# ecpoppenheimer/TensorFlowRayTrace

Measured on AMD Instinct MI355X. Metric: ray-surface intersection tests/sec (fwd+bwd), higher is better.
Workload: dtype f32 ray state, f32 filter + f64 decisions

## Files before the change

### tensorflowraytrace_amd/csrc/tfrt_trace3d.hip

```cpp
#include <vector>

#include <type_traits>
#include "tfrt_common.h"
#include "goal_finish.h"
#include "wave_schedule.h"

namespace tfrt {

constexpr int TILE = 512;
constexpr int KC = 24;

constexpr int ERR_CAPACITY = 1;


__global__ __launch_bounds__(BLOCK) void k_center(const double* __restrict__ fverts, int M,
                                                  double* __restrict__ c0, int32_t* nrays0, int n,
                                                  int32_t* tail8, unsigned int* scan_ticket) {
  if (nrays0 != nullptr) {
    if (threadIdx.x == 0) *nrays0 = n;
    if (threadIdx.x < 8) tail8[threadIdx.x] = 0;
    if (threadIdx.x == 0 && scan_ticket != nullptr) *scan_ticket = 0u;
  }
  __shared__ double red[WAVES][3];
  __shared__ double ctr[3];
// ... 2473 lines not shown
  if (p == a.P && a.P > 0 && a.unfinished != nullptr) {
    const unsigned long long m = __ballot(alive);
    if (alive) {
      const int slot = a.wbase[(size_t)(a.P - 1) * a.wstride + qwave].x + rank_below(m);
      const T* rin = a.rays_ws + (size_t)(a.P - 1) * 6 * a.n;
#pragma unroll
      for (int k = 0; k < 6; ++k) a.unfinished[(int64_t)k * a.N + slot] = rin[k * a.n + i];
      if (a.unfinished_id != nullptr) a.unfinished_id[slot] = rid;
    }
  }
}


template <typename G>
__device__ __forceinline__ void add6(const G* g, int64_t cap, int64_t slot, double a[3],
                                     double b[3]) {
  if (g == nullptr) return;
  for (int k = 0; k < 3; ++k) {
    a[k] += static_cast<double>(g[k * cap + slot]);
    b[k] += static_cast<double>(g[(3 + k) * cap + slot]);
  }
}

template <typename T>
struct SweepStore {
  using type = float;
};
template <>
struct SweepStore<double> {
  using type = double;
};

template <typename T>
__device__ __forceinline__ int backward_ray(
    int i, const T* __restrict__ rays_in, int64_t stride_in, const int32_t* __restrict__ ray_id_in,
    const int32_t* __restrict__ rec_tri, const double* __restrict__ rec_t,
    const uint8_t* __restrict__ rec_cls, const int32_t* __restrict__ rec_slot,
    const int32_t* __restrict__ pass_counts, const tfrt_scene3d& sc, double L, double dead_len,
    const typename SweepStore<T>::type* __restrict__ g_child, int64_t child_stride,
    const double* __restrict__ g_fin, int64_t cap_fin, const double* __restrict__ g_act,
    int64_t cap_act, const double* __restrict__ g_stp, int64_t cap_stp,
    const double* __restrict__ g_dead, int64_t cap_dead,
    typename SweepStore<T>::type* __restrict__ g_out, double* __restrict__ g_src_out,
    int64_t out_stride, double gP[9]);

template <int CTRL>
__device__ __forceinline__ double dpp_f64(const double v) {
  const long long b = __double_as_longlong(v);
  const int lo = __builtin_amdgcn_update_dpp(0, (int)(b & 0xFFFFFFFFll), CTRL, 0xF, 0xF, false);
  const int hi = __builtin_amdgcn_update_dpp(0, (int)(b >> 32), CTRL, 0xF, 0xF, false);
  return __longlong_as_double(((long long)hi << 32) | (unsigned int)lo);
}

constexpr int WSUM_SLOTS = 32, WSUM_CELLS = 576;
__device__ __forceinline__ void wave_face_sums(int tri, const double gP[9], double* wacc,
                                               int32_t* wface, double* __restrict__ g_fverts) {
  const int lane = threadIdx.x & 63;
  int slot = -1, ns = 0;
  unsigned long long todo = __ballot(tri >= 0);
  if (todo == 0ull) return;
  while (todo != 0ull && ns < WSUM_SLOTS) {
    const int leader = __ffsll((long long)todo) - 1;
    const int k = __builtin_amdgcn_readlane(tri, leader);
    const bool mine = tri == k;
    if (mine) slot = ns;
    if (lane == leader) wface[ns] = k;
    ++ns;
    todo &= ~__ballot(mine);
  }
  const int copies = ns <= 8 ? 8 : (ns <= 16 ? 4 : 2);
  const int cells = ns * 9 * copies;
  for (int k = lane; k < cells; k += 64) wacc[k] = 0.0;
  wave_fence();
  if (tri >= 0) {
    if (slot >= 0) {
      double* w = &wacc[slot * 9 * copies + (lane & (copies - 1))];
#pragma unroll
      for (int c = 0; c < 9; ++c)
        if (gP[c] != 0.0) unsafeAtomicAdd(w + c * copies, gP[c]);
    } else {
      double* gp = g_fverts + 9 * (int64_t)tri;
#pragma unroll
      for (int c = 0; c < 9; ++c)
        if (gP[c] != 0.0) unsafeAtomicAdd(gp + c, gP[c]);
    }
  }
  wave_fence();
  for (int k0 = 0; k0 < cells; k0 += 64) {
    const int k = k0 + lane;
    double v = k < cells ? wacc[k] : 0.0;
    v += dpp_f64<0xB1>(v);
    if (copies >= 4) v += dpp_f64<0x4E>(v);
    if (copies >= 8) v += dpp_f64<0x141>(v);
    if ((lane & (copies - 1)) == 0 && k < cells && v != 0.0) {
      const int term = k / copies;
      unsafeAtomicAdd(g_fverts + 9 * (int64_t)wface[term / 9] + (term % 9), v);
    }
  }
  wave_fence();
}

template <typename T, int BW>
__global__ __launch_bounds__(64 * BW) void k_backward3d(
    const T* __restrict__ rays_in, int64_t stride_in, const int32_t* __restrict__ n_ptr,
    const int32_t* __restrict__ ray_id_in, const int32_t* __restrict__ rec_tri,
    const double* __restrict__ rec_t, const uint8_t* __restrict__ rec_cls,
    const int32_t* __restrict__ rec_slot, const int32_t* __restrict__ pass_counts,
    tfrt_scene3d sc, double L, double dead_len,
    const typename SweepStore<T>::type* __restrict__ g_child, int64_t child_stride,
    const double* __restrict__ g_fin, int64_t cap_fin, const double* __restrict__ g_act,
    int64_t cap_act, const double* __restrict__ g_stp, int64_t cap_stp,
    const double* __restrict__ g_dead, int64_t cap_dead,
    typename SweepStore<T>::type* __restrict__ g_out, double* __restrict__ g_src_out,
    int64_t out_stride, double* __restrict__ g_fverts,
    typename SweepStore<T>::type* __restrict__ stash_g, int32_t* __restrict__ stash_face,
    int wave_sums) {
  const int n = *n_ptr;
  const int q0 = blockIdx.x * (64 * BW) + threadIdx.x;
  const int i = q0;
  if (wave_sums) {
    if ((q0 & ~63) >= n) return;
    __shared__ double wacc[BW][WSUM_CELLS];
    __shared__ int32_t wface[BW][WSUM_SLOTS];
    const int wave = threadIdx.x >> 6;
    double gP[9];
    int tri = -1;
    if (i < n)
      tri = backward_ray<T>(i, rays_in, stride_in, ray_id_in, rec_tri, rec_t, rec_cls, rec_slot,
                            pass_counts, sc, L, dead_len, g_child, child_stride, g_fin, cap_fin,
                            g_act, cap_act, g_stp, cap_stp, g_dead, cap_dead, g_out, g_src_out,
                            out_stride, gP);
    wave_face_sums(tri, gP, wacc[wave], wface[wave], g_fverts);
    return;
  }
  if (i >= n) return;
  double gP[9];
  const int tri = backward_ray<T>(i, rays_in, stride_in, ray_id_in, rec_tri, rec_t, rec_cls,
                                  rec_slot, pass_counts, sc, L, dead_len, g_child, child_stride,
                                  g_fin, cap_fin, g_act, cap_act, g_stp, cap_stp, g_dead, cap_dead,
                                  g_out, g_src_out, out_stride, gP);
  if (stash_face != nullptr) {
    stash_face[i] = tri;
    if (tri >= 0) {
      using S = typename SweepStore<T>::type;
      S* o = stash_g + 9 * (int64_t)i;
#pragma unroll
      for (int c = 0; c < 9; ++c) o[c] = static_cast<S>(gP[c]);
    }
    return;
  }
  if (tri >= 0) {
    double* gp = g_fverts + 9 * (int64_t)tri;
#pragma unroll
    for (int c = 0; c < 9; ++c) {
      if (gP[c] != 0.0) unsafeAtomicAdd(gp + c, gP[c]);
    }
  }
}

constexpr int FACE_WINDOW = 2048;

template <typename S>
__global__ __launch_bounds__(1024) void k_face_accumulate(
    const int32_t* __restrict__ nrays, int passes, int64_t pass_stride,
    const int32_t* __restrict__ stash_face, const S* __restrict__ stash_g, int chunk, int M,
    double* __restrict__ g_fverts) {
  __shared__ double acc[FACE_WINDOW * 9];
  const int lo = blockIdx.x * chunk;
  if (lo >= nrays[0]) return;
  const int w0 = blockIdx.y * FACE_WINDOW;
  const int w1 = min(M, w0 + FACE_WINDOW);
  for (int k = threadIdx.x; k < FACE_WINDOW * 9; k += 1024) acc[k] = 0.0;
  __syncthreads();
  for (int p = 0; p < passes; ++p) {
    const int hi = min(nrays[p], lo + chunk);
    const int32_t* __restrict__ face = stash_face + (int64_t)p * pass_stride;
    const S* __restrict__ terms = stash_g + 9 * (int64_t)p * pass_stride;
// ... 152 lines not shown
      const double dl = (dead_len != 0.0) ? dead_len : 1.0;
      for (int k = 0; k < 3; ++k) {
        gs[k] = a[k] + (1.0 - dl) * b[k];
        ge[k] = dl * b[k];
      }
    }
  } else {
    double g_s[3] = {0, 0, 0}, g_h[3] = {0, 0, 0}, g_ce[3] = {0, 0, 0};
    bool has_child = false;
    if (cls == CLS_FINISHED) {
      if (seed_fin != nullptr) {
        for (int k = 0; k < 3; ++k) {
          g_s[k] += seed_fin[k];
          g_h[k] += seed_fin[3 + k];
        }
      } else {
        add6(g_fin, cap_fin, slot, g_s, g_h);
      }
    } else if (cls == CLS_STOPPED) {
      add6(g_stp, cap_stp, slot, g_s, g_h);
    } else {
      if (g_act != nullptr)
        add6(g_act, cap_act, (slot_global ? 0 : (int64_t)pass_counts[4 + CLS_ACTIVE]) + slot, g_s, g_h);
      if (child_pass) {
        has_child = true;
        for (int k = 0; k < 3; ++k) {
          g_h[k] += child[k];
          g_ce[k] += child[3 + k];
        }
      }
    }
    bool nz = has_child;
    for (int k = 0; k < 3; ++k) nz = nz || g_s[k] != 0.0 || g_h[k] != 0.0;
    if (nz) {
      if (!early) {
        if (tri_known < -1) tri = rec_tri[i];
        load_face(has_child);
      }
      double gn[2];
      const bool want_n = GN && has_child && sc.grad_n_in != nullptr && sc.n_table == nullptr;
      const int branch = ((tape & TAPE_INTERNAL) ? 1 : 0) | ((tape & TAPE_REFLECT) ? 2 : 0);
      adjoint3d(s, e, P, t_rec, has_child, n_in, n_out, L, g_s, g_h, g_ce, gs, ge, gP, gn, branch,
                want_n);
      if (want_n) {
        if (gn[0] != 0.0) unsafeAtomicAdd(sc.grad_n_in + tri, gn[0]);
        if (gn[1] != 0.0) unsafeAtomicAdd(sc.grad_n_out + tri, gn[1]);
      }
      if (sc.face_grad_mask == nullptr || sc.face_grad_mask[tri] != 0) face_out = tri;
    }
  }
  return face_out;
}

__device__ __forceinline__ int backward_core_loaded(
    int tape, int tri, bool child_pass, const double s[3], const double e[3], const double P[9],
    double t_rec, double n_in, double n_out, bool face_wanted, double L, const double child[6],
    const double seed[6], double gs[3], double ge[3], double gP[9]) {
  int face_out = -1;
  const int cls = tape & 3;
  for (int k = 0; k < 3; ++k) gs[k] = ge[k] = 0.0;
  if (cls != CLS_DEAD) {
    double g_s[3] = {0, 0, 0}, g_h[3] = {0, 0, 0}, g_ce[3] = {0, 0, 0};
    bool has_child = false;
    if (cls == CLS_FINISHED) {
      for (int k = 0; k < 3; ++k) {
        g_s[k] += seed[k];
        g_h[k] += seed[3 + k];
      }
    } else if (cls == CLS_ACTIVE && child_pass) {
      has_child = true;
      for (int k = 0; k < 3; ++k) {
        g_h[k] += child[k];
        g_ce[k] += child[3 + k];
      }
    }
    bool nz = has_child;
    for (int k = 0; k < 3; ++k) nz = nz || g_s[k] != 0.0 || g_h[k] != 0.0;
    if (nz) {
      const int branch = ((tape & TAPE_INTERNAL) ? 1 : 0) | ((tape & TAPE_REFLECT) ? 2 : 0);
      adjoint3d(s, e, P, t_rec, has_child, n_in, n_out, L, g_s, g_h, g_ce, gs, ge, gP, nullptr,
                branch, false);
      if (face_wanted) face_out = tri;
    }
  }
  return face_out;
}

template <typename T>
__device__ __forceinline__ int backward_ray(
    int i, const T* __restrict__ rays_in, int64_t stride_in, const int32_t* __restrict__ ray_id_in,
    const int32_t* __restrict__ rec_tri, const double* __restrict__ rec_t,
    const uint8_t* __restrict__ rec_cls, const int32_t* __restrict__ rec_slot,
    const int32_t* __restrict__ pass_counts, const tfrt_scene3d& sc, double L, double dead_len,
    const typename SweepStore<T>::type* __restrict__ g_child, int64_t child_stride,
    const double* __restrict__ g_fin, int64_t cap_fin, const double* __restrict__ g_act,
    int64_t cap_act, const double* __restrict__ g_stp, int64_t cap_stp,
    const double* __restrict__ g_dead, int64_t cap_dead,
    typename SweepStore<T>::type* __restrict__ g_out, double* __restrict__ g_src_out,
    int64_t out_stride, double gP[9]) {
  const int tape = rec_cls[i];
  const int slot = rec_slot[i];
  double child[6] = {0, 0, 0, 0, 0, 0};
  const bool child_pass = g_child != nullptr;
  if (child_pass && (tape & 3) == CLS_ACTIVE) {
    for (int k = 0; k < 6; ++k) child[k] = static_cast<double>(g_child[k * child_stride + slot]);
  }
  double gs[3], ge[3];
  const int face_out = backward_core<T>(i, tape, slot, rays_in, stride_in, ray_id_in, rec_tri,
                                        rec_t, pass_counts, sc, L, dead_len, child_pass, child,
                                        nullptr, g_fin, cap_fin, g_act, cap_act, g_stp, cap_stp, g_dead,
                                        cap_dead, gs, ge, gP);
  if (g_out != nullptr) {
    using G = typename SweepStore<T>::type;
    for (int k = 0; k < 3; ++k) {
      g_out[k * out_stride + i] = static_cast<G>(gs[k]);
      g_out[(3 + k) * out_stride + i] = static_cast<G>(ge[k]);
    }
  } else if (g_src_out != nullptr) {
    for (int k = 0; k < 3; ++k) {
      g_src_out[k * out_stride + i] = gs[k];
      g_src_out[(3 + k) * out_stride + i] = ge[k];
    }
  }
  return face_out;
}

constexpr int CHAIN_MAXP = 8;

template <typename T>
struct ChainArgs {
  const T* src;
  int64_t src_stride;
  const T* rays_ws;
  const int32_t* nrays;
  const int32_t* rayid;
  const int32_t* rec_tri;
  const int32_t* rec_slot;
  const double* rec_t;
  const uint8_t* rec_cls;
  const int32_t* counts;
  int64_t n;
  int32_t P;
  double L, dead_len;
  const double *g_fin, *g_act, *g_stp, *g_dead;
  int64_t cap_fin, cap_act, cap_stp, cap_dead;
  double* g_src;
  int64_t N;
  double* g_fverts;
  const T* fin_rays;
  int64_t fin_cap;
  GoalFields gf;
  const double* goal;
  int64_t goal_stride, goal_ray_stride;
  double* partial;
  int32_t* partial_cnt;
  const double* feta;
  int32_t inplace;
  int32_t chain_in_lds;
};

#ifndef TFRT_CHAIN_WAVES
#define TFRT_CHAIN_WAVES 4
#endif
template <typename T, int BW, bool GOAL, bool GN>
__global__ __launch_bounds__(64 * BW)
__attribute__((amdgpu_waves_per_eu(TFRT_CHAIN_WAVES, TFRT_CHAIN_WAVES))) void k_backward_chain(
    ChainArgs<T> a, tfrt_scene3d sc) {
#pragma clang fp contract(off)
  const int n0 = a.nrays[0];
  const int i0 = blockIdx.x * (64 * BW) + threadIdx.x;
  if ((i0 & ~63) >= n0) {
    if (GOAL && (threadIdx.x & 63) == 0) {
      a.partial[i0 >> 6] = 0.0;
      if (a.partial_cnt != nullptr) a.partial_cnt[2 * (i0 >> 6)] = a.partial_cnt[2 * (i0 >> 6) + 1] = 0;
    }
    return;
  }
  __shared__ double wacc[BW][WSUM_CELLS];
  __shared__ int32_t wface[BW][WSUM_SLOTS];
  extern __shared__ int4 chain_lds[];
  const int lane = threadIdx.x & 63, wave = threadIdx.x >> 6;
  const int P = a.P;
  int4* chain = chain_lds + (size_t)wave * P * 64;
  int last = -1;
  if (i0 < n0) {
    int j = i0;
    for (int p = 0; p < P; ++p) {
      const size_t at = (size_t)p * a.n + j;
      const int tape = a.rec_cls[at], tri = a.rec_tri[at];
      const int slot = a.inplace >= 2 ? j : a.rec_slot[at];
      if (a.chain_in_lds) chain[p * 64 + lane] = make_int4(j, tape, slot, tri);
      last = p;
      if ((tape & 3) != CLS_ACTIVE || p == P - 1) break;
      if (!a.inplace) j = slot;
    }
  }
  int top = last;
#pragma unroll
  for (int d = 32; d > 0; d >>= 1) top = max(top, __shfl_xor(top, d, 64));
  double child[6] = {0, 0, 0, 0, 0, 0};
  double err = 0.0;
  int n_fin = 0, n_entered = 0;
  for (int p = top; p >= 0; --p) {
    double gP[9];
    int tri = -1;
    bool fin_here = false;
    if (p <= last) {
      int4 rec;
      if (a.chain_in_lds) {
        rec = chain[p * 64 + lane];
      } else {
        const size_t at = (size_t)p * a.n + i0;
        rec = make_int4(i0, a.rec_cls[at], a.inplace >= 2 ? i0 : a.rec_slot[at], a.rec_tri[at]);
      }
      const int j = rec.x, tape = rec.y, slot = rec.z;
      const size_t off = (size_t)p * a.n;
      const T* rin = p == 0 ? a.src : a.rays_ws + (size_t)(p - 1) * 6 * a.n;
      const int64_t sin = p == 0 ? a.src_stride : a.n;
      const int32_t* idin = (p == 0 || a.inplace) ? nullptr : a.rayid + (size_t)(p - 1) * a.n;
      double seed[6] = {0, 0, 0, 0, 0, 0};
      if (GOAL && p == last && (tape & 3) == CLS_FINISHED) {
        fin_here = true;
        double fin_row[6] = {0, 0, 0, 0, 0, 0};
        if (a.inplace) {
          double s0[3], e0[3], h0[3];
          load_ray3(rin, sin, j, s0, e0);
          hit_point(s0, e0, a.rec_t[off + j], h0);
#pragma unroll
          for (int k = 0; k < 3; ++k) {
            fin_row[k] = s0[k];
            fin_row[3 + k] = static_cast<double>(static_cast<T>(h0[k]));
          }
        }
        for (int c = 0; c < a.gf.n; ++c) {
          const int row = a.gf.row[c];
          double out_c = 0.0;
// ... 21 lines not shown
                             rec.w, a.feta, a.inplace != 0);
      for (int k = 0; k < 3; ++k) {
        child[k] = gs[k];
        child[3 + k] = ge[k];
      }
    }
    if (GOAL) {
      n_fin += __popcll(__ballot(fin_here));
      n_entered += __popcll(__ballot(p <= last));
    }
    wave_face_sums(tri, gP, wacc[wave], wface[wave], a.g_fverts);
  }
  if (a.g_src != nullptr && i0 < n0) {
    for (int k = 0; k < 6; ++k) a.g_src[k * a.N + i0] = child[k];
  }
  if (GOAL) {
#pragma unroll
    for (int d = 32; d > 0; d >>= 1) err += __shfl_xor(err, d, 64);
    if (lane == 0) {
      a.partial[i0 >> 6] = err;
      if (a.partial_cnt != nullptr) {
        a.partial_cnt[2 * (i0 >> 6)] = n_fin;
        a.partial_cnt[2 * (i0 >> 6) + 1] = n_entered;
      }
    }
  }
}

template <typename T>
struct ChainGoalArgs {
  const T* src;
  int64_t src_stride;
  const T* rays_ws;
  const int32_t* nrays;
  const int32_t* rec_tri;
  const double* rec_t;
  const uint8_t* rec_cls;
  int64_t n;
  int32_t P;
  double L;
  double* g_src;
  int64_t N;
  double* g_fverts;
  GoalFields gf;
  const double* goal;
  int64_t goal_stride, goal_ray_stride;
  double* partial;
  int32_t* partial_cnt;
  const double* feta;
  const double* face_verts;
  const uint8_t* face_grad_mask;
  const int32_t* sched;
  int32_t ngroups;
};

template <typename T>
__global__ __launch_bounds__(64)
__attribute__((amdgpu_waves_per_eu(TFRT_CHAIN_WAVES, TFRT_CHAIN_WAVES))) void k_backward_chain_goal_inplace(
    ChainGoalArgs<T> a) {
#pragma clang fp contract(off)
  const int n0 = a.nrays[0];
  int wave = blockIdx.x;
  if (a.sched != nullptr) {
    wave = __builtin_amdgcn_readfirstlane(a.sched[blockIdx.x]);
    if ((unsigned)wave >= (unsigned)a.ngroups) return;
  }
  const int i0 = wave * 64 + threadIdx.x;
  const int lane = threadIdx.x;
  if ((i0 & ~63) >= n0) {
    if (lane == 0) {
      a.partial[i0 >> 6] = 0.0;
      if (a.partial_cnt != nullptr) a.partial_cnt[2 * (i0 >> 6)] = a.partial_cnt[2 * (i0 >> 6) + 1] = 0;
    }
    return;
  }
  __builtin_assume(a.feta != nullptr);
  __shared__ double wacc[WSUM_CELLS];
  __shared__ int32_t wface[WSUM_SLOTS];
  extern __shared__ int2 chain_goal_lds[];
  int2* chain = chain_goal_lds;
  const int P = a.P;
  int last = -1;
  if (i0 < n0) {
    for (int p = 0; p < P; ++p) {
      const size_t at = (size_t)p * a.n + i0;
      const int tape = a.rec_cls[at], tri = a.rec_tri[at];
      chain[p * 64 + lane] = make_int2(tape, tri);
      last = p;
      if ((tape & 3) != CLS_ACTIVE) break;
    }
  }
  int top = last;
#pragma unroll
  for (int d = 32; d > 0; d >>= 1) top = max(top, __shfl_xor(top, d, 64));
  top = __builtin_amdgcn_readfirstlane(top);
  double child[6] = {0, 0, 0, 0, 0, 0};
  double err = 0.0;
  int n_fin = 0, n_entered = 0;
  for (int p = top; p >= 0; --p) {
    double gP[9];
    int tri = -1;
    bool fin_here = false;
    if (p <= last) {
      const int2 rec = chain[p * 64 + lane];
      const int tape = rec.x, cls = tape & 3;
      const int face = max(rec.y, -1);
      const size_t off = (size_t)p * a.n;
      const T* rin = p == 0 ? a.src : a.rays_ws + (size_t)(p - 1) * 6 * a.n;
      const int64_t sin = p == 0 ? a.src_stride : a.n;
      const bool child_pass = p < P - 1;
      fin_here = p == last && cls == CLS_FINISHED;
      const bool on_face = face >= 0 && cls != CLS_DEAD;
      const bool with_child = on_face && child_pass && cls == CLS_ACTIVE;
      int iv = i0;
      __asm__ volatile("" : "+v"(iv));
      T ray_w[6];
#pragma unroll
      for (int k = 0; k < 6; ++k) ray_w[k] = rin[k * sin + iv];
      double t_rec = 0.0;
      if (fin_here || on_face) t_rec = a.rec_t[off + iv];
      double goal_w[6];
#pragma unroll
      for (int c = 0; c < 6; ++c) {
        goal_w[c] = 0.0;
        if (fin_here && c < a.gf.n)
          goal_w[c] = a.goal[(int64_t)c * a.goal_stride + (int64_t)iv * a.goal_ray_stride];
      }
      double Pf[9] = {0, 0, 0, 0, 0, 0, 0, 0, 0}, n_in = 1.0, n_out = 1.0;
      uint8_t mask_w = 1;
      if (on_face) {
        const double* fp = a.face_verts + 9 * (int64_t)face;
#pragma unroll
        for (int q = 0; q < 9; ++q) Pf[q] = fp[q];
        if (a.face_grad_mask != nullptr && (with_child || cls == CLS_FINISHED))
          mask_w = a.face_grad_mask[face];
      }
      if (with_child) {
        n_in = a.feta[4 * (int64_t)face + 2];
        n_out = a.feta[4 * (int64_t)face + 3];
      }
      double s0[3], e0[3];
#pragma unroll
      for (int k = 0; k < 3; ++k) {
        s0[k] = static_cast<double>(ray_w[k]);
        e0[k] = static_cast<double>(ray_w[3 + k]);
      }
      int mask_i = mask_w;
      __asm__ volatile("" : "+v"(mask_i));
      double seed[6] = {0, 0, 0, 0, 0, 0};
      if (fin_here) {
        double fin_row[6], h0[3];
        hit_point(s0, e0, t_rec, h0);
#pragma unroll
        for (int k = 0; k < 3; ++k) {
          fin_row[k] = s0[k];
          fin_row[3 + k] = static_cast<double>(static_cast<T>(h0[k]));
        }
#pragma nounroll
        for (int c = 0; c < a.gf.n; ++c) {
          const int row = a.gf.row[c];
          double out_c = 0.0, goal_c = 0.0;
#pragma unroll
          for (int k = 0; k < 6; ++k) {
            if (k == row) out_c = fin_row[k];
            if (k == c) goal_c = goal_w[k];
          }
          const double r = out_c - goal_c;
          const double g = 2.0 * r;
#pragma unroll
          for (int q = 0; q < 6; ++q)
            if (q == row) seed[q] = g;
          err += r * r;
        }
      }
      double gs[3], ge[3];
      tri = backward_core_loaded(tape, face, child_pass, s0, e0, Pf, t_rec, n_in, n_out,
                                 mask_i != 0, a.L, child, seed, gs, ge, gP);
      for (int k = 0; k < 3; ++k) {
        child[k] = gs[k];
        child[3 + k] = ge[k];
      }
    }
    n_fin += __popcll(__ballot(fin_here));
    n_entered += __popcll(__ballot(p <= last));
    wave_face_sums(tri, gP, wacc, wface, a.g_fverts);
  }
  if (a.g_src != nullptr && i0 < n0) {
    for (int k = 0; k < 6; ++k) a.g_src[k * a.N + i0] = child[k];
  }
#pragma unroll
  for (int d = 32; d > 0; d >>= 1) err += __shfl_xor(err, d, 64);
  if (lane == 0) {
    a.partial[i0 >> 6] = err;
    if (a.partial_cnt != nullptr) {
      a.partial_cnt[2 * (i0 >> 6)] = n_fin;
      a.partial_cnt[2 * (i0 >> 6) + 1] = n_entered;
    }
  }
}


template <typename T>
__global__ __launch_bounds__(BLOCK) void k_finalize_seam(
    const T* __restrict__ rays, int64_t stride, int n, int chunks,
    const double* __restrict__ part_t, const int32_t* __restrict__ part_i, int64_t part_stride,
    const double* __restrict__ fverts, int M, double eps_int, double eps_size, double eps_start,
    double* x, double* y, double* z, uint8_t* valid, double* ray_u, double* trig_u,
    double* trig_v, int32_t* gather_trig) {
  const int i = blockIdx.x * BLOCK + threadIdx.x;
  if (i >= n) return;
  double bt = INFINITY;
  int bi = -1;
  for (int c = 0; c < chunks; ++c) {
    const double t = part_t[c * part_stride + i];
    if (t < bt) {
      bt = t;
      bi = part_i[c * part_stride + i];
    }
  }
  const int tri = bi < 0 ? 0 : bi;
  double s[3], e[3], P[9], h[3] = {0, 0, 0};
  TriHit th;
  th.ray_u = th.trig_u = th.trig_v = 0.0;
  th.valid = false;
  if (M > 0) {
    load_ray3(rays, stride, i, s, e);
    for (int q = 0; q < 9; ++q) P[q] = fverts[9 * (int64_t)tri + q];
    th = exact_triangle(s, e, P, eps_int, eps_size, eps_start);
    hit_point(s, e, th.ray_u, h);
  }
  x[i] = h[0];
  y[i] = h[1];
  z[i] = h[2];
  valid[i] = bi >= 0;
  ray_u[i] = bi >= 0 ? th.ray_u : INFINITY;
  trig_u[i] = th.trig_u;
  trig_v[i] = th.trig_v;
// ... 598 lines not shown
    if (inplace && sc->in_place == 2 &&
        (c.g_act || c.g_stp || c.g_dead || c.goal != nullptr || c.cap_fin < N))
      return TFRT_E_BADARG;
    a.inplace = !inplace ? 0
                : (sc->in_place == 2 ? 3
                   : ((c.g_fin || c.g_act || c.g_stp || c.g_dead || c.goal == nullptr) ? 1 : 2));
    a.chain_in_lds = P <= CHAIN_MAXP ? 1 : 0;
    a.fin_rays = nullptr;
    a.fin_cap = 0;
    a.gf.n = 0;
    a.goal = nullptr;
    a.goal_stride = a.goal_ray_stride = 0;
    a.partial = nullptr;
    a.partial_cnt = nullptr;
    a.feta = per_face_indices(sc) ? tape.feta : nullptr;
    const size_t chain_lds = a.chain_in_lds ? (size_t)P * 64 * sizeof(int4) : 0;
    ProfScope prof_bwd(TFRT_PROF_BACKWARD, st);
    if (c.goal != nullptr) {
      a.fin_rays = static_cast<const T*>(c.goal->fin_rays);
      a.fin_cap = c.goal->fin_cap;
      a.gf = c.goal->gf;
      a.goal = c.goal->goal;
      a.goal_stride = c.goal->goal_stride;
      a.goal_ray_stride = c.goal->goal_ray_stride;
      a.partial = c.goal->partial;
      a.partial_cnt = c.goal->partial_cnt;
      if (N > 0 && a.inplace == 2 && a.chain_in_lds && a.feta != nullptr &&
          sc->grad_n_in == nullptr) {
        ChainGoalArgs<T> g;
        g.src = a.src;
        g.src_stride = a.src_stride;
        g.rays_ws = a.rays_ws;
        g.nrays = a.nrays;
        g.rec_tri = a.rec_tri;
        g.rec_t = a.rec_t;
        g.rec_cls = a.rec_cls;
        g.n = a.n;
        g.P = a.P;
        g.L = a.L;
        g.g_src = a.g_src;
        g.N = a.N;
        g.g_fverts = a.g_fverts;
        g.gf = a.gf;
        g.goal = a.goal;
        g.goal_stride = a.goal_stride;
        g.goal_ray_stride = a.goal_ray_stride;
        g.partial = a.partial;
        g.partial_cnt = a.partial_cnt;
        g.feta = a.feta;
        g.face_verts = sc->face_verts;
        g.face_grad_mask = sc->face_grad_mask;
        g.sched = sc->wave_schedule;
        g.ngroups = cdiv(N, 64);
        hipLaunchKernelGGL((k_backward_chain_goal_inplace<T>), dim3(cdiv(N, 64)), dim3(64),
                           (size_t)P * 64 * sizeof(int2), st, g);
      } else if (N > 0 && sc->grad_n_in != nullptr)
        hipLaunchKernelGGL((k_backward_chain<T, 1, true, true>), dim3(cdiv(N, 64)), dim3(64),
                           chain_lds, st, a, *sc);
      else if (N > 0)
        hipLaunchKernelGGL((k_backward_chain<T, 1, true, false>), dim3(cdiv(N, 64)), dim3(64),
                           chain_lds, st, a, *sc);
    } else if (N > 0 && sc->grad_n_in != nullptr) {
      hipLaunchKernelGGL((k_backward_chain<T, 1, false, true>), dim3(cdiv(N, 64)), dim3(64),
                         chain_lds, st, a, *sc);
    } else if (N > 0) {
      hipLaunchKernelGGL((k_backward_chain<T, 1, false, false>), dim3(cdiv(N, 64)), dim3(64),
                         chain_lds, st, a, *sc);
    }
    return hipGetLastError() == hipSuccess ? 0 : TFRT_E_LAUNCH;
  }
  for (int p = P - 1; p >= 0; --p) {
    const PassIn<T> in = tape.input(p, c.src, c.src_stride);
    const G* g_child = (p == P - 1) ? nullptr : gbuf + (size_t)((p + 1) & 1) * 6 * n;
    G* g_out = p == 0 ? nullptr : gbuf + (size_t)(p & 1) * 6 * n;
    double* g_src_out = p == 0 ? c.g_src : nullptr;
    const int64_t out_stride = p == 0 ? N : n;
    G* stash_g = stash_g_all + (size_t)p * 9 * n;
    int32_t* stash_face = stash_face_all + (size_t)p * n;
    ProfScope prof_bwd(TFRT_PROF_BACKWARD, st);
    constexpr int BWD_BW = 1;
    hipLaunchKernelGGL((k_backward3d<T, BWD_BW>), dim3(cdiv(N, 64 * BWD_BW)), dim3(64 * BWD_BW), 0,
                       st, in.rays, in.stride, nrays + p, in.ids, tape.rec_tri(p), tape.rec_t(p),
                       tape.rec_cls(p), tape.rec_slot(p),
                       c.counts + (size_t)p * TFRT_COUNTS_PER_PASS, *sc, c.L, c.dead_len, g_child,
                       n, c.g_fin, c.cap_fin, c.g_act, c.cap_act, c.g_stp, c.cap_stp,
                       c.g_dead, c.cap_dead, g_out, g_src_out, out_stride, c.g_fverts,
                       stash ? stash_g : nullptr, stash ? stash_face : nullptr, wave_sums ? 1 : 0);
    if (ordered) {
      unsigned long long* mx = fix_max + ((P - 1 - p) & 1);
      hipLaunchKernelGGL((k_stash_absmax<G>), dim3(pl.nblk), dim3(BLOCK), 0, st, nrays + p, stash_face,
                         stash_g, mx);
      hipLaunchKernelGGL((k_face_accumulate_fixed<G>), dim3(pl.nblk), dim3(BLOCK), 0, st, nrays + p,
                         stash_face, stash_g, mx, fix_acc, fix_flag);
      hipLaunchKernelGGL(k_fixed_finish, dim3(cdiv((int64_t)M * 9, BLOCK)), dim3(BLOCK), 0, st,
                         (int64_t)M * 9, mx, fix_max + (((P - 1 - p) & 1) ^ 1), fix_acc,
                         fix_flag, c.g_fverts);
    }
  }
  if (stash && !ordered && P > 0) {
    ProfScope prof_acc(TFRT_PROF_ACCUMULATE, st);
    hipLaunchKernelGGL((k_face_accumulate<G>), dim3(cdiv(N, acc_chunk), windows), dim3(1024), 0, st,
                       nrays, P, n, stash_face_all, stash_g_all, acc_chunk, M, c.g_fverts);
  }
  return hipGetLastError() == hipSuccess ? 0 : TFRT_E_LAUNCH;
}

// ... 298 lines not shown
```

### tensorflowraytrace_amd/csrc/trace_math.h

```cpp
#pragma once
#include <math.h>

#if defined(__HIPCC__)
#define TFRT_HD __host__ __device__ __forceinline__
#else
#define TFRT_HD inline
#endif

namespace tfrt {

constexpr int CLS_ACTIVE = 0;
constexpr int CLS_FINISHED = 1;
constexpr int CLS_STOPPED = 2;
constexpr int CLS_DEAD = 3;

constexpr int CAT_OPTICAL = 0, CAT_STOP = 1, CAT_TARGET = 2;

struct TriHit {
  double ray_u, trig_u, trig_v;
  bool valid;
};

TFRT_HD TriHit exact_triangle(const double s[3], const double e[3], const double P[9],
                              double eps_int, double eps_size, double eps_start) {
// ... 137 lines not shown

TFRT_HD double fmod_floor(double x, double m) {
  double r = fmod(x, m);
  if (r != 0.0 && ((r < 0.0) != (m < 0.0))) r += m;
  return r;
}

TFRT_HD double snell2d_angle(double xs, double ys, double xe, double ye, double norm,
                             double n_in, double n_out) {
#pragma clang fp contract(off)
  const double PI = 3.141592653589793;
  norm = fmod_floor(norm, 2 * PI);
  double ray_angle = atan2(ys - ye, xs - xe);
  ray_angle = fmod_floor(ray_angle, 2 * PI);
  double theta1 = norm - ray_angle;
  if (theta1 > PI) theta1 = theta1 - 2 * PI;
  if (theta1 < -PI) theta1 = theta1 + 2 * PI;
  const bool internal = fabs(theta1) >= PI / 2;
  const bool in_safe = n_in != 0.0, out_safe = n_out != 0.0;
  const double nis = in_safe ? n_in : 1.0, nos = out_safe ? n_out : 1.0;
  const double n1 = out_safe ? nis / nos : 0.0;
  const double n2 = in_safe ? nos / nis : 0.0;
  const double n = internal ? n1 : n2;
  if (!internal) norm = norm + PI;
  if (internal) theta1 = theta1 + PI;
  const double theta2 = n * sin(theta1);
  if (fabs(theta2) <= 1.0 && n != 0.0) return norm - asin(theta2);
  return norm + theta1 + PI;
}

TFRT_HD double adj_rcp(double x) {
#if defined(__HIP_DEVICE_COMPILE__)
  double r = __builtin_amdgcn_rcp(x);
  r = __builtin_fma(__builtin_fma(-x, r, 1.0), r, r);
  r = __builtin_fma(__builtin_fma(-x, r, 1.0), r, r);
  return r;
#else
  return 1.0 / x;
#endif
}
TFRT_HD double adj_rsqrt(double x) {
#if defined(__HIP_DEVICE_COMPILE__)
  double y = __builtin_amdgcn_rsq(x);
  double e = __builtin_fma(-x * y, y, 1.0);
  y = __builtin_fma(0.5 * y, e, y);
  e = __builtin_fma(-x * y, y, 1.0);
  y = __builtin_fma(0.5 * y, e, y);
  return y;
#else
  return 1.0 / sqrt(x);
#endif
}

TFRT_HD void adjoint3d(const double s[3], const double e[3], const double P[9], double ray_u,
                       bool has_child, double n_in, double n_out, double L,
                       const double g_s[3], const double g_h[3], const double g_ce[3],
                       double gs[3], double ge[3], double gP[9], double* gn = nullptr,
                       int branch = -1, bool gn_wanted = true) {
  if (gn != nullptr) gn[0] = gn[1] = 0.0;
  const double d[3] = {e[0] - s[0], e[1] - s[1], e[2] - s[2]};
  const double E1[3] = {P[3] - P[0], P[4] - P[1], P[5] - P[2]};
  const double E2[3] = {P[6] - P[0], P[7] - P[1], P[8] - P[2]};
  double C[3];
  cross3(E1, E2, C);
  const double t = ray_u;
  double h[3] = {s[0] + t * d[0], s[1] + t * d[1], s[2] + t * d[2]};

  double hb[3] = {g_h[0], g_h[1], g_h[2]};
  double sb[3] = {g_s[0], g_s[1], g_s[2]};
  double Cn[3] = {0.0, 0.0, 0.0};

  if (has_child) {
    const double inv_c = adj_rsqrt(dot3(C, C));
    const double n[3] = {C[0] * inv_c, C[1] * inv_c, C[2] * inv_c};
    const double r[3] = {h[0] - s[0], h[1] - s[1], h[2] - s[2]};
    const double rsq = dot3(r, r);
    const bool clamped = rsq < 1e-12;
    const double inv_r = clamped ? 1e6 : adj_rsqrt(rsq);
    const double u[3] = {r[0] * inv_r, r[1] * inv_r, r[2] * inv_r};
    const double nu = dot3(n, u);
    const bool in_safe = n_in != 0.0, out_safe = n_out != 0.0;
    const double nis = in_safe ? n_in : 1.0, nos = out_safe ? n_out : 1.0;
    const bool internal = branch >= 0 ? (branch & 1) != 0 : nu > 0.0;
    const double eta = internal ? (out_safe ? nis / nos : 0.0) : (in_safe ? nos / nis : 0.0);
    const double nu_eta = eta * nu;
    double k = 1.0 - eta * eta + nu_eta * nu_eta;
    const bool reflect = branch >= 0 ? (branch & 2) != 0 : ((k < 0.0) || (n_in == 0.0));
    if (!reflect && k < 0.0) k = 0.0;
    double wb[3], ub[3], nb[3];
    for (int i = 0; i < 3; ++i) {
      hb[i] += g_ce[i];
      wb[i] = L * g_ce[i];
    }
    double nub;
    if (reflect) {
      nub = -2.0 * dot3(wb, n);
      for (int i = 0; i < 3; ++i) {
        ub[i] = wb[i];
        nb[i] = -2.0 * nu * wb[i];
      }
    } else {
      const double sg = branch >= 0 ? (internal ? 1.0 : (nu < 0.0 ? -1.0 : 0.0))
                                    : ((nu > 0.0) ? 1.0 : ((nu < 0.0) ? -1.0 : 0.0));
      const double irk = k > 0.0 ? adj_rsqrt(k) : INFINITY;
      const double rk = k > 0.0 ? k * irk : 0.0;
      const double alpha = sg * rk - nu_eta;
      const double ab = dot3(wb, n);
      nub = ab * (sg * eta * nu_eta * irk - eta);
      if (gn != nullptr && gn_wanted) {
        const double etab = dot3(wb, u) + ab * (sg * eta * (nu * nu - 1.0) * irk - nu);
        if (internal) {
          if (out_safe) {
            gn[0] = in_safe ? etab / nos : 0.0;
            gn[1] = -etab * eta / nos;
          }
        } else if (in_safe) {
          gn[1] = out_safe ? etab / nis : 0.0;
          gn[0] = -etab * eta / nis;
        }
      }
      for (int i = 0; i < 3; ++i) {
        nb[i] = alpha * wb[i];
        ub[i] = eta * wb[i];
      }
    }
    for (int i = 0; i < 3; ++i) {
      nb[i] += nub * u[i];
      ub[i] += nub * n[i];
    }
    if (!clamped) {
      const double uu = dot3(u, ub);
      for (int i = 0; i < 3; ++i) {
        const double rb = (ub[i] - u[i] * uu) * inv_r;
        hb[i] += rb;
        sb[i] -= rb;
      }
    } else {
      for (int i = 0; i < 3; ++i) {
        hb[i] += ub[i] * 1e6;
        sb[i] -= ub[i] * 1e6;
      }
    }
    const double nn = dot3(n, nb);
    for (int i = 0; i < 3; ++i) Cn[i] = (nb[i] - n[i] * nn) * inv_c;
  }

  double db[3];
  double tb = 0.0;
  for (int i = 0; i < 3; ++i) {
    sb[i] += hb[i];
    tb += hb[i] * d[i];
    db[i] = t * hb[i];
  }
  const double den = dot3(d, C);
  const double numb = tb * adj_rcp(den);
  const double denb = -numb * t;
  double Cb[3];
  for (int i = 0; i < 3; ++i) {
    sb[i] -= numb * C[i];
    Cb[i] = Cn[i] + (numb * (P[i] - s[i]) + denb * d[i]);
    db[i] += denb * C[i];
  }
  double E1b[3], E2b[3];
  cross3(E2, Cb, E1b);
  cross3(Cb, E1, E2b);
  for (int i = 0; i < 3; ++i) {
    gP[3 + i] = E1b[i];
    gP[6 + i] = E2b[i];
    gP[i] = numb * C[i] - (E1b[i] + E2b[i]);
    ge[i] = db[i];
    gs[i] = sb[i] - db[i];
  }
}

}
```

Measured before the change: 126400 billion.

## Restructure backward chain-goal pass with copy-major face sums, role split, eta table

Reworks the per-wave face-gradient accumulator into a copy-major LDS layout that is cleared once per kernel and folded and re-zeroed in place, replacing the per-step clear and DPP reduction. Splits the chain-goal backward pass into finished-role and child-role template instances, using scalar-base loads and precomputed goal-column mappings when goal rows are ascending. Passes precomputed refraction ratios from the feta table instead of dividing indices. Skips face-gradient terms when the face is masked out, and contracts the adjoint dot and cross products into explicit FMAs. These changes aim to cut LDS traffic, divisions, divergence and ALU work in the backward pass, at the cost of more code paths and slightly different floating-point rounding.

```diff
diff --git a/tensorflowraytrace_amd/csrc/tfrt_trace3d.hip b/tensorflowraytrace_amd/csrc/tfrt_trace3d.hip
--- a/tensorflowraytrace_amd/csrc/tfrt_trace3d.hip
+++ b/tensorflowraytrace_amd/csrc/tfrt_trace3d.hip
@@ -2549,7 +2549,41 @@
   return __longlong_as_double(((long long)hi << 32) | (unsigned int)lo);
 }
 
+#ifndef TFRT_SWEEP_COPY_MAJOR
+#define TFRT_SWEEP_COPY_MAJOR 1
+#endif
+#if TFRT_SWEEP_COPY_MAJOR
+constexpr int WSUM_SLOTS = 32, WSUM_CELLS = 592;
+__device__ __forceinline__ constexpr int wsum_stride(int copies) {
+  return WSUM_SLOTS * 9 * 2 / copies + 2;
+}
+static_assert(8 * wsum_stride(8) <= WSUM_CELLS && 4 * wsum_stride(4) <= WSUM_CELLS &&
+              2 * wsum_stride(2) <= WSUM_CELLS, "wacc holds every tier");
+
+__device__ __forceinline__ void wsum_clear(double* wacc) {
+  for (int k = 2 * (threadIdx.x & 63); k < WSUM_CELLS; k += 128)
+    *reinterpret_cast<double2*>(wacc + k) = make_double2(0.0, 0.0);
+  wave_fence();
+}
+template <int COPIES>
+__device__ __forceinline__ void wsum_fold(double* wacc, const int32_t* wface, int K, int lane,
+                                          double* __restrict__ g_fverts) {
+  for (int k = lane; k < K; k += 64) {
+    double* w = wacc + k;
+    double v = w[0];
+#pragma unroll
+    for (int c = 1; c < COPIES; ++c) v += w[c * wsum_stride(COPIES)];
+#pragma unroll
+    for (int c = 0; c < COPIES; ++c) w[c * wsum_stride(COPIES)] = 0.0;
+    if (v != 0.0) {
+      const int f = k / 9;
+      unsafeAtomicAdd(g_fverts + 9 * (int64_t)wface[f] + (k - 9 * f), v);
+    }
+  }
+}
+#else
 constexpr int WSUM_SLOTS = 32, WSUM_CELLS = 576;
+#endif
 __device__ __forceinline__ void wave_face_sums(int tri, const double gP[9], double* wacc,
                                                int32_t* wface, double* __restrict__ g_fverts) {
   const int lane = threadIdx.x & 63;
@@ -2565,6 +2599,27 @@
     ++ns;
     todo &= ~__ballot(mine);
   }
+#if TFRT_SWEEP_COPY_MAJOR
+  const int copies = ns <= 8 ? 8 : (ns <= 16 ? 4 : 2);
+  if (tri >= 0) {
+    if (slot >= 0) {
+      double* w = &wacc[(lane & (copies - 1)) * wsum_stride(copies) + slot * 9];
+#pragma unroll
+      for (int c = 0; c < 9; ++c)
+        if (gP[c] != 0.0) unsafeAtomicAdd(w + c, gP[c]);
+    } else {
+      double* gp = g_fverts + 9 * (int64_t)tri;
+#pragma unroll
+      for (int c = 0; c < 9; ++c)
+        if (gP[c] != 0.0) unsafeAtomicAdd(gp + c, gP[c]);
+    }
+  }
+  wave_fence();
+  if (copies == 8) wsum_fold<8>(wacc, wface, ns * 9, lane, g_fverts);
+  else if (copies == 4) wsum_fold<4>(wacc, wface, ns * 9, lane, g_fverts);
+  else wsum_fold<2>(wacc, wface, ns * 9, lane, g_fverts);
+  wave_fence();
+#else
   const int copies = ns <= 8 ? 8 : (ns <= 16 ? 4 : 2);
   const int cells = ns * 9 * copies;
   for (int k = lane; k < cells; k += 64) wacc[k] = 0.0;
@@ -2595,6 +2650,7 @@
     }
   }
   wave_fence();
+#endif
 }
 
 template <typename T, int BW>
@@ -2617,9 +2673,12 @@
   const int i = q0;
   if (wave_sums) {
     if ((q0 & ~63) >= n) return;
-    __shared__ double wacc[BW][WSUM_CELLS];
+    __shared__ __align__(16) double wacc[BW][WSUM_CELLS];
     __shared__ int32_t wface[BW][WSUM_SLOTS];
     const int wave = threadIdx.x >> 6;
+#if TFRT_SWEEP_COPY_MAJOR
+    wsum_clear(wacc[wave]);
+#endif
     double gP[9];
     int tri = -1;
     if (i < n)
@@ -2878,9 +2937,16 @@
   return face_out;
 }
 
+#ifndef TFRT_SWEEP_SKIP_FROZEN
+#define TFRT_SWEEP_SKIP_FROZEN 1
+#endif
+#ifndef TFRT_SWEEP_ETA_TABLE
+#define TFRT_SWEEP_ETA_TABLE 1
+#endif
+template <bool FIN = true, bool CHILD = true>
 __device__ __forceinline__ int backward_core_loaded(
     int tape, int tri, bool child_pass, const double s[3], const double e[3], const double P[9],
-    double t_rec, double n_in, double n_out, bool face_wanted, double L, const double child[6],
+    double t_rec, double n_a, double n_b, bool face_wanted, double L, const double child[6],
     const double seed[6], double gs[3], double ge[3], double gP[9]) {
   int face_out = -1;
   const int cls = tape & 3;
@@ -2888,12 +2954,12 @@
   if (cls != CLS_DEAD) {
     double g_s[3] = {0, 0, 0}, g_h[3] = {0, 0, 0}, g_ce[3] = {0, 0, 0};
     bool has_child = false;
-    if (cls == CLS_FINISHED) {
+    if (FIN && cls == CLS_FINISHED) {
       for (int k = 0; k < 3; ++k) {
         g_s[k] += seed[k];
         g_h[k] += seed[3 + k];
       }
-    } else if (cls == CLS_ACTIVE && child_pass) {
+    } else if (CHILD && cls == CLS_ACTIVE && child_pass) {
       has_child = true;
       for (int k = 0; k < 3; ++k) {
         g_h[k] += child[k];
@@ -2904,8 +2970,15 @@
     for (int k = 0; k < 3; ++k) nz = nz || g_s[k] != 0.0 || g_h[k] != 0.0;
     if (nz) {
       const int branch = ((tape & TAPE_INTERNAL) ? 1 : 0) | ((tape & TAPE_REFLECT) ? 2 : 0);
-      adjoint3d(s, e, P, t_rec, has_child, n_in, n_out, L, g_s, g_h, g_ce, gs, ge, gP, nullptr,
-                branch, false);
+      const bool face_terms = TFRT_SWEEP_SKIP_FROZEN ? face_wanted : true;
+#if TFRT_SWEEP_ETA_TABLE
+      const double ratios[2] = {n_a, n_b};
+      adjoint3d(s, e, P, t_rec, has_child, 1.0, 1.0, L, g_s, g_h, g_ce, gs, ge, gP, nullptr,
+                branch, false, face_terms, ratios);
+#else
+      adjoint3d(s, e, P, t_rec, has_child, n_a, n_b, L, g_s, g_h, g_ce, gs, ge, gP, nullptr,
+                branch, false, face_terms);
+#endif
       if (face_wanted) face_out = tri;
     }
   }
@@ -3002,12 +3075,15 @@
     }
     return;
   }
-  __shared__ double wacc[BW][WSUM_CELLS];
+  __shared__ __align__(16) double wacc[BW][WSUM_CELLS];
   __shared__ int32_t wface[BW][WSUM_SLOTS];
   extern __shared__ int4 chain_lds[];
   const int lane = threadIdx.x & 63, wave = threadIdx.x >> 6;
   const int P = a.P;
   int4* chain = chain_lds + (size_t)wave * P * 64;
+#if TFRT_SWEEP_COPY_MAJOR
+  wsum_clear(wacc[wave]);
+#endif
   int last = -1;
   if (i0 < n0) {
     int j = i0;
@@ -3135,7 +3211,158 @@
   const uint8_t* face_grad_mask;
   const int32_t* sched;
   int32_t ngroups;
+  int32_t goal_col[6];
+  uint32_t rows_packed;
+  int32_t rows_ascending;
 };
+
+#ifndef TFRT_SWEEP_ROLES
+#define TFRT_SWEEP_ROLES 1
+#endif
+#ifndef TFRT_SWEEP_GOAL_ROWS
+#define TFRT_SWEEP_GOAL_ROWS 1
+#endif
+
+template <typename T>
+static void chain_goal_columns(ChainGoalArgs<T>& g) {
+  bool asc = TFRT_SWEEP_GOAL_ROWS != 0;
+  for (int c = 1; c < g.gf.n; ++c) asc = asc && g.gf.row[c] > g.gf.row[c - 1];
+  g.rows_ascending = asc ? 1 : 0;
+  g.rows_packed = 0;
+  for (int j = 0; j < 6; ++j) g.goal_col[j] = (!asc && j < g.gf.n) ? j : -1;
+  for (int c = 0; c < g.gf.n; ++c) {
+    g.rows_packed |= (uint32_t)(g.gf.row[c] & 7) << (4 * c);
+    if (asc) g.goal_col[g.gf.row[c]] = c;
+  }
+}
+
+template <typename U>
+__device__ __forceinline__ U ld_scalar_base(const U* base, unsigned long long byte_offset) {
+  unsigned long long v = reinterpret_cast<unsigned long long>(base);
+  __asm__ volatile("" : "+s"(v));
+  typedef const U __attribute__((address_space(1))) G;
+  return *reinterpret_cast<G*>(v + byte_offset);
+}
+template <typename U>
+__device__ __forceinline__ U ld_lane(const U* base, uint32_t i) {
+  return ld_scalar_base(base, (unsigned long long)(i * (uint32_t)sizeof(U)));
+}
+
+template <typename T, bool FIN, bool CHILD>
+__device__ __forceinline__ int chain_goal_pass(const ChainGoalArgs<T>& a, int p, int wave, int lane,
+                                               int tape, int face, bool fin_lane, double child[6],
+                                               double& err, double gP[9]) {
+#pragma clang fp contract(off)
+  const int cls = tape & 3;
+  const size_t off = (size_t)p * a.n;
+  const T* rin = p == 0 ? a.src : a.rays_ws + (size_t)(p - 1) * 6 * a.n;
+  const int64_t sin = p == 0 ? a.src_stride : a.n;
+  const bool child_pass = CHILD && p < a.P - 1;
+  const bool fin_here = FIN && fin_lane;
+  const bool on_face = face >= 0 && cls != CLS_DEAD;
+  const bool with_child = on_face && child_pass && cls == CLS_ACTIVE;
+  T ray_w[6];
+  double t_rec = 0.0;
+  double goal_w[6] = {0, 0, 0, 0, 0, 0};
+#if TFRT_SWEEP_ROLES
+  uint32_t lv = lane;
+  __asm__ volatile("" : "+v"(lv));
+  const size_t w0 = (size_t)wave * 64;
+#pragma unroll
+  for (int k = 0; k < 6; ++k) ray_w[k] = ld_lane(rin + k * sin + w0, lv);
+  if (fin_here || on_face) t_rec = ld_lane(a.rec_t + off + w0, lv);
+  if (FIN) {
+    const int64_t gl = (int64_t)lv * a.goal_ray_stride;
+#pragma unroll
+    for (int j = 0; j < 6; ++j) {
+      int cj = a.goal_col[j];
+      __asm__ volatile("" : "+s"(cj));
+      if (cj >= 0) {
+        const double* gb = a.goal + (int64_t)cj * a.goal_stride + (int64_t)w0 * a.goal_ray_stride;
+        if (fin_here) goal_w[j] = ld_scalar_base(gb, (unsigned long long)gl * sizeof(double));
+      }
+    }
+  }
+#else
+  int iv = wave * 64 + lane;
+  __asm__ volatile("" : "+v"(iv));
+#pragma unroll
+  for (int k = 0; k < 6; ++k) ray_w[k] = rin[k * sin + iv];
+  if (fin_here || on_face) t_rec = a.rec_t[off + iv];
+#pragma unroll
+  for (int j = 0; j < 6; ++j) {
+    const int cj = a.goal_col[j];
+    if (FIN && cj >= 0 && fin_here)
+      goal_w[j] = a.goal[(int64_t)cj * a.goal_stride + (int64_t)iv * a.goal_ray_stride];
+  }
+#endif
+  double Pf[9] = {0, 0, 0, 0, 0, 0, 0, 0, 0}, n_a = 1.0, n_b = 1.0;
+  uint8_t mask_w = 1;
+  if (on_face) {
+    const double* fp = a.face_verts + 9 * (int64_t)face;
+#pragma unroll
+    for (int q = 0; q < 9; ++q) Pf[q] = fp[q];
+    if (a.face_grad_mask != nullptr && (with_child || (FIN && cls == CLS_FINISHED)))
+      mask_w = a.face_grad_mask[face];
+  }
+  if (with_child) {
+    n_a = a.feta[4 * (int64_t)face + (TFRT_SWEEP_ETA_TABLE ? 0 : 2)];
+    n_b = a.feta[4 * (int64_t)face + (TFRT_SWEEP_ETA_TABLE ? 1 : 3)];
+  }
+  double s0[3], e0[3];
+#pragma unroll
+  for (int k = 0; k < 3; ++k) {
+    s0[k] = static_cast<double>(ray_w[k]);
+    e0[k] = static_cast<double>(ray_w[3 + k]);
+  }
+  int mask_i = mask_w;
+  __asm__ volatile("" : "+v"(mask_i));
+  double seed[6] = {0, 0, 0, 0, 0, 0};
+  if (fin_here) {
+    double fin_row[6], h0[3];
+    hit_point(s0, e0, t_rec, h0);
+#pragma unroll
+    for (int k = 0; k < 3; ++k) {
+      fin_row[k] = s0[k];
+      fin_row[3 + k] = static_cast<double>(static_cast<T>(h0[k]));
+    }
+    if (a.rows_ascending) {
+#pragma unroll
+      for (int k = 0; k < 6; ++k) {
+        if (a.goal_col[k] >= 0) {
+          const double r = fin_row[k] - goal_w[k];
+          seed[k] = 2.0 * r;
+          err += r * r;
+        }
+      }
+    } else {
+#pragma nounroll
+      for (int c = 0; c < a.gf.n; ++c) {
+        const int row = (a.rows_packed >> (4 * c)) & 7;
+        double out_c = 0.0, goal_c = 0.0;
+#pragma unroll
+        for (int k = 0; k < 6; ++k) {
+          if (k == row) out_c = fin_row[k];
+          if (k == c) goal_c = goal_w[k];
+        }
+        const double r = out_c - goal_c;
+        const double g = 2.0 * r;
+#pragma unroll
+        for (int q = 0; q < 6; ++q)
+          if (q == row) seed[q] = g;
+        err += r * r;
+      }
+    }
+  }
+  double gs[3], ge[3];
+  const int tri = backward_core_loaded<FIN, CHILD>(tape, face, child_pass, s0, e0, Pf, t_rec, n_a,
+                                                   n_b, mask_i != 0, a.L, child, seed, gs, ge, gP);
+  for (int k = 0; k < 3; ++k) {
+    child[k] = gs[k];
+    child[3 + k] = ge[k];
+  }
+  return tri;
+}
 
 template <typename T>
 __global__ __launch_bounds__(64)
@@ -3158,10 +3385,13 @@
     return;
   }
   __builtin_assume(a.feta != nullptr);
-  __shared__ double wacc[WSUM_CELLS];
+  __shared__ __align__(16) double wacc[WSUM_CELLS];
   __shared__ int32_t wface[WSUM_SLOTS];
   extern __shared__ int2 chain_goal_lds[];
   int2* chain = chain_goal_lds;
+#if TFRT_SWEEP_COPY_MAJOR
+  wsum_clear(wacc);
+#endif
   const int P = a.P;
   int last = -1;
   if (i0 < n0) {
@@ -3183,89 +3413,27 @@
   for (int p = top; p >= 0; --p) {
     double gP[9];
     int tri = -1;
-    bool fin_here = false;
-    if (p <= last) {
+    const bool here = p <= last;
+    int tape = CLS_DEAD, face = -1;
+    if (here) {
       const int2 rec = chain[p * 64 + lane];
-      const int tape = rec.x, cls = tape & 3;
-      const int face = max(rec.y, -1);
-      const size_t off = (size_t)p * a.n;
-      const T* rin = p == 0 ? a.src : a.rays_ws + (size_t)(p - 1) * 6 * a.n;
-      const int64_t sin = p == 0 ? a.src_stride : a.n;
-      const bool child_pass = p < P - 1;
-      fin_here = p == last && cls == CLS_FINISHED;
-      const bool on_face = face >= 0 && cls != CLS_DEAD;
-      const bool with_child = on_face && child_pass && cls == CLS_ACTIVE;
-      int iv = i0;
-      __asm__ volatile("" : "+v"(iv));
-      T ray_w[6];
-#pragma unroll
-      for (int k = 0; k < 6; ++k) ray_w[k] = rin[k * sin + iv];
-      double t_rec = 0.0;
-      if (fin_here || on_face) t_rec = a.rec_t[off + iv];
-      double goal_w[6];
-#pragma unroll
-      for (int c = 0; c < 6; ++c) {
-        goal_w[c] = 0.0;
-        if (fin_here && c < a.gf.n)
-          goal_w[c] = a.goal[(int64_t)c * a.goal_stride + (int64_t)iv * a.goal_ray_stride];
-      }
-      double Pf[9] = {0, 0, 0, 0, 0, 0, 0, 0, 0}, n_in = 1.0, n_out = 1.0;
-      uint8_t mask_w = 1;
-      if (on_face) {
-        const double* fp = a.face_verts + 9 * (int64_t)face;
-#pragma unroll
-        for (int q = 0; q < 9; ++q) Pf[q] = fp[q];
-        if (a.face_grad_mask != nullptr && (with_child || cls == CLS_FINISHED))
-          mask_w = a.face_grad_mask[face];
-      }
-      if (with_child) {
-        n_in = a.feta[4 * (int64_t)face + 2];
-        n_out = a.feta[4 * (int64_t)face + 3];
-      }
-      double s0[3], e0[3];
-#pragma unroll
-      for (int k = 0; k < 3; ++k) {
-        s0[k] = static_cast<double>(ray_w[k]);
-        e0[k] = static_cast<double>(ray_w[3 + k]);
-      }
-      int mask_i = mask_w;
-      __asm__ volatile("" : "+v"(mask_i));
-      double seed[6] = {0, 0, 0, 0, 0, 0};
-      if (fin_here) {
-        double fin_row[6], h0[3];
-        hit_point(s0, e0, t_rec, h0);
-#pragma unroll
-        for (int k = 0; k < 3; ++k) {
-          fin_row[k] = s0[k];
-          fin_row[3 + k] = static_cast<double>(static_cast<T>(h0[k]));
-        }
-#pragma nounroll
-        for (int c = 0; c < a.gf.n; ++c) {
-          const int row = a.gf.row[c];
-          double out_c = 0.0, goal_c = 0.0;
-#pragma unroll
-          for (int k = 0; k < 6; ++k) {
-            if (k == row) out_c = fin_row[k];
-            if (k == c) goal_c = goal_w[k];
-          }
-          const double r = out_c - goal_c;
-          const double g = 2.0 * r;
-#pragma unroll
-          for (int q = 0; q < 6; ++q)
-            if (q == row) seed[q] = g;
-          err += r * r;
-        }
-      }
-      double gs[3], ge[3];
-      tri = backward_core_loaded(tape, face, child_pass, s0, e0, Pf, t_rec, n_in, n_out,
-                                 mask_i != 0, a.L, child, seed, gs, ge, gP);
-      for (int k = 0; k < 3; ++k) {
-        child[k] = gs[k];
-        child[3 + k] = ge[k];
-      }
-    }
-    n_fin += __popcll(__ballot(fin_here));
-    n_entered += __popcll(__ballot(p <= last));
+      tape = rec.x;
+      face = max(rec.y, -1);
+    }
+    const bool fin_here = here && p == last && (tape & 3) == CLS_FINISHED;
+    const unsigned long long fin_m = __ballot(fin_here);
+#if TFRT_SWEEP_ROLES
+    const bool fin_role = here && fin_m != 0ull && !(p < P - 1 && (tape & 3) == CLS_ACTIVE);
+    if (fin_role)
+      tri = chain_goal_pass<T, true, false>(a, p, wave, lane, tape, face, fin_here, child, err, gP);
+    if (here && !fin_role)
+      tri = chain_goal_pass<T, false, true>(a, p, wave, lane, tape, face, false, child, err, gP);
+#else
+    if (here)
+      tri = chain_goal_pass<T, true, true>(a, p, wave, lane, tape, face, fin_here, child, err, gP);
+#endif
+    n_fin += __popcll(fin_m);
+    n_entered += __popcll(__ballot(here));
     wave_face_sums(tri, gP, wacc, wface, a.g_fverts);
   }
   if (a.g_src != nullptr && i0 < n0) {
@@ -3970,6 +4138,7 @@
         g.face_grad_mask = sc->face_grad_mask;
         g.sched = sc->wave_schedule;
         g.ngroups = cdiv(N, 64);
+        chain_goal_columns(g);
         hipLaunchKernelGGL((k_backward_chain_goal_inplace<T>), dim3(cdiv(N, 64)), dim3(64),
                            (size_t)P * 64 * sizeof(int2), st, g);
       } else if (N > 0 && sc->grad_n_in != nullptr)
diff --git a/tensorflowraytrace_amd/csrc/trace_math.h b/tensorflowraytrace_amd/csrc/trace_math.h
--- a/tensorflowraytrace_amd/csrc/trace_math.h
+++ b/tensorflowraytrace_amd/csrc/trace_math.h
@@ -213,17 +213,38 @@
 #endif
 }
 
+#ifndef TFRT_ADJ_CONTRACT
+#define TFRT_ADJ_CONTRACT 1
+#endif
+TFRT_HD double adj_dot3(const double a[3], const double b[3]) {
+#if defined(__HIP_DEVICE_COMPILE__) && TFRT_ADJ_CONTRACT
+  return __builtin_fma(a[2], b[2], __builtin_fma(a[1], b[1], a[0] * b[0]));
+#else
+  return dot3(a, b);
+#endif
+}
+TFRT_HD void adj_cross3(const double a[3], const double b[3], double o[3]) {
+#if defined(__HIP_DEVICE_COMPILE__) && TFRT_ADJ_CONTRACT
+  o[0] = __builtin_fma(a[1], b[2], -(a[2] * b[1]));
+  o[1] = __builtin_fma(a[2], b[0], -(a[0] * b[2]));
+  o[2] = __builtin_fma(a[0], b[1], -(a[1] * b[0]));
+#else
+  cross3(a, b, o);
+#endif
+}
+
 TFRT_HD void adjoint3d(const double s[3], const double e[3], const double P[9], double ray_u,
                        bool has_child, double n_in, double n_out, double L,
                        const double g_s[3], const double g_h[3], const double g_ce[3],
                        double gs[3], double ge[3], double gP[9], double* gn = nullptr,
-                       int branch = -1, bool gn_wanted = true) {
+                       int branch = -1, bool gn_wanted = true, bool face_terms = true,
+                       const double* ratios = nullptr) {
   if (gn != nullptr) gn[0] = gn[1] = 0.0;
   const double d[3] = {e[0] - s[0], e[1] - s[1], e[2] - s[2]};
   const double E1[3] = {P[3] - P[0], P[4] - P[1], P[5] - P[2]};
   const double E2[3] = {P[6] - P[0], P[7] - P[1], P[8] - P[2]};
   double C[3];
-  cross3(E1, E2, C);
+  adj_cross3(E1, E2, C);
   const double t = ray_u;
   double h[3] = {s[0] + t * d[0], s[1] + t * d[1], s[2] + t * d[2]};
 
@@ -232,18 +253,20 @@
   double Cn[3] = {0.0, 0.0, 0.0};
 
   if (has_child) {
-    const double inv_c = adj_rsqrt(dot3(C, C));
+    const double inv_c = adj_rsqrt(adj_dot3(C, C));
     const double n[3] = {C[0] * inv_c, C[1] * inv_c, C[2] * inv_c};
     const double r[3] = {h[0] - s[0], h[1] - s[1], h[2] - s[2]};
-    const double rsq = dot3(r, r);
+    const double rsq = adj_dot3(r, r);
     const bool clamped = rsq < 1e-12;
     const double inv_r = clamped ? 1e6 : adj_rsqrt(rsq);
     const double u[3] = {r[0] * inv_r, r[1] * inv_r, r[2] * inv_r};
-    const double nu = dot3(n, u);
+    const double nu = adj_dot3(n, u);
     const bool in_safe = n_in != 0.0, out_safe = n_out != 0.0;
     const double nis = in_safe ? n_in : 1.0, nos = out_safe ? n_out : 1.0;
     const bool internal = branch >= 0 ? (branch & 1) != 0 : nu > 0.0;
-    const double eta = internal ? (out_safe ? nis / nos : 0.0) : (in_safe ? nos / nis : 0.0);
+    const double eta = ratios != nullptr
+                           ? (internal ? ratios[0] : ratios[1])
+                           : (internal ? (out_safe ? nis / nos : 0.0) : (in_safe ? nos / nis : 0.0));
     const double nu_eta = eta * nu;
     double k = 1.0 - eta * eta + nu_eta * nu_eta;
     const bool reflect = branch >= 0 ? (branch & 2) != 0 : ((k < 0.0) || (n_in == 0.0));
@@ -255,7 +278,7 @@
     }
     double nub;
     if (reflect) {
-      nub = -2.0 * dot3(wb, n);
+      nub = -2.0 * adj_dot3(wb, n);
       for (int i = 0; i < 3; ++i) {
         ub[i] = wb[i];
         nb[i] = -2.0 * nu * wb[i];
@@ -266,10 +289,10 @@
       const double irk = k > 0.0 ? adj_rsqrt(k) : INFINITY;
       const double rk = k > 0.0 ? k * irk : 0.0;
       const double alpha = sg * rk - nu_eta;
-      const double ab = dot3(wb, n);
+      const double ab = adj_dot3(wb, n);
       nub = ab * (sg * eta * nu_eta * irk - eta);
       if (gn != nullptr && gn_wanted) {
-        const double etab = dot3(wb, u) + ab * (sg * eta * (nu * nu - 1.0) * irk - nu);
+        const double etab = adj_dot3(wb, u) + ab * (sg * eta * (nu * nu - 1.0) * irk - nu);
         if (internal) {
           if (out_safe) {
             gn[0] = in_safe ? etab / nos : 0.0;
@@ -290,7 +313,7 @@
       ub[i] += nub * n[i];
     }
     if (!clamped) {
-      const double uu = dot3(u, ub);
+      const double uu = adj_dot3(u, ub);
       for (int i = 0; i < 3; ++i) {
         const double rb = (ub[i] - u[i] * uu) * inv_r;
         hb[i] += rb;
@@ -302,8 +325,10 @@
         sb[i] -= ub[i] * 1e6;
       }
     }
-    const double nn = dot3(n, nb);
-    for (int i = 0; i < 3; ++i) Cn[i] = (nb[i] - n[i] * nn) * inv_c;
+    if (face_terms) {
+      const double nn = adj_dot3(n, nb);
+      for (int i = 0; i < 3; ++i) Cn[i] = (nb[i] - n[i] * nn) * inv_c;
+    }
   }
 
   double db[3];
@@ -313,22 +338,24 @@
     tb += hb[i] * d[i];
     db[i] = t * hb[i];
   }
-  const double den = dot3(d, C);
+  const double den = adj_dot3(d, C);
   const double numb = tb * adj_rcp(den);
   const double denb = -numb * t;
-  double Cb[3];
+  if (face_terms) {
+    double Cb[3];
+    for (int i = 0; i < 3; ++i) Cb[i] = Cn[i] + (numb * (P[i] - s[i]) + denb * d[i]);
+    double E1b[3], E2b[3];
+    adj_cross3(E2, Cb, E1b);
+    adj_cross3(Cb, E1, E2b);
+    for (int i = 0; i < 3; ++i) {
+      gP[3 + i] = E1b[i];
+      gP[6 + i] = E2b[i];
+      gP[i] = numb * C[i] - (E1b[i] + E2b[i]);
+    }
+  }
   for (int i = 0; i < 3; ++i) {
     sb[i] -= numb * C[i];
-    Cb[i] = Cn[i] + (numb * (P[i] - s[i]) + denb * d[i]);
     db[i] += denb * C[i];
-  }
-  double E1b[3], E2b[3];
-  cross3(E2, Cb, E1b);
-  cross3(Cb, E1, E2b);
-  for (int i = 0; i < 3; ++i) {
-    gP[3 + i] = E1b[i];
-    gP[6 + i] = E2b[i];
-    gP[i] = numb * C[i] - (E1b[i] + E2b[i]);
     ge[i] = db[i];
     gs[i] = sb[i] - db[i];
   }
```

Measured after the change: 130200 billion (median of 6 runs). 1.03x the previous value.
